# Mbed-TLS/mbedtls

Hardware: AMD Instinct MI355X
Metric: TLS records/sec + GiB/s AEAD throughput (device-resident), 16 KiB records (higher is better)
Workload: dtype u8

## Files before the change

### mbedtls_amd/csrc/tlsrec_device.h

```cpp
#ifndef TLSREC_DEVICE_H
#define TLSREC_DEVICE_H

#include <hip/hip_runtime.h>
#include <stdint.h>

namespace tlsrec {

struct SboxGen {
    uint8_t v[256];
    constexpr SboxGen() : v() {
        uint8_t ex[256] = {};
        uint8_t lg[256] = {};
        uint8_t x = 1;
        for (int i = 0; i < 255; i++) {
            ex[i] = x;
            lg[x] = (uint8_t) i;
            uint8_t x2 = (uint8_t) ((x << 1) ^ ((x & 0x80) ? 0x1b : 0));
            x = (uint8_t) (x2 ^ x);
        }
        for (int a = 0; a < 256; a++) {
            uint8_t inv = a ? ex[(255 - lg[a]) % 255] : 0;
            uint8_t s = inv, r = inv;
            for (int k = 0; k < 4; k++) {
                r = (uint8_t) ((r << 1) | (r >> 7));
// ... 318 lines not shown
        return cam_encrypt<NR, OFF>(lds, lb, rk, in);
    else
        return aria_encrypt<NR, OFF>(lds, lb, rk, in);
}

template <int NR, bool ARIA, typename RK>
__device__ __forceinline__ uint4 blk_encrypt(const uint8_t *lds, uint32_t lb, RK rk, uint4 in)
{
    if constexpr (ARIA)
        return alt_encrypt<NR, 0>(lds, lb, rk, in);
    else
        return aes_encrypt<NR, 0>(lds, lb, rk, in);
}

template <int PI, int G = 4, bool MEM = true>
__device__ __forceinline__ uint4 gmul(const uint8_t *lds, uint4 y)
{
    const uint32_t w[4] = { y.x, y.y, y.z, y.w };
    uint4 acc = make_uint4(0, 0, 0, 0);
#pragma unroll
    for (int d = 0; d < 4; d++) {
#pragma unroll
        for (int e = 0; e < 4; e++) {
            const int b = 4 * d + e;
            uint32_t ahi = (e == 0) ? (w[d] & 0xf0u) : ((w[d] >> (8 * e)) & 0xf0u);
            uint32_t alo = (e == 0) ? ((w[d] << 4) & 0xf0u) : ((w[d] >> (8 * e - 4)) & 0xf0u);
            uint4 th = *reinterpret_cast<const uint4 *>(lds + ahi + PI * 8192 + (2 * b) * 256);
            uint4 tl = *reinterpret_cast<const uint4 *>(lds + alo + PI * 8192 + (2 * b + 1) * 256);
            acc.x = xor3(acc.x, th.x, tl.x);
            acc.y = xor3(acc.y, th.y, tl.y);
            acc.z = xor3(acc.z, th.z, tl.z);
            acc.w = xor3(acc.w, th.w, tl.w);
        }
        if ((d + 1) % (4 / G) == 0) {
            if constexpr (MEM)
                asm volatile("" : "+v"(acc.x), "+v"(acc.y), "+v"(acc.z), "+v"(acc.w) : : "memory");
            else
                asm volatile("" : "+v"(acc.x), "+v"(acc.y), "+v"(acc.z), "+v"(acc.w));
        }
    }
    return acc;
}

template <int PI, int NE = 4>
__device__ __forceinline__ void gmul_word(const uint8_t *lds, uint32_t wd, int d, uint4 &acc, int e0 = 0)
{
#pragma unroll
    for (int i = 0; i < NE; i++) {
        const int e = e0 + i;
        const int b = 4 * d + e;
        uint32_t ahi = (e == 0) ? (wd & 0xf0u) : ((wd >> (8 * e)) & 0xf0u);
        uint32_t alo = (e == 0) ? ((wd << 4) & 0xf0u) : ((wd >> (8 * e - 4)) & 0xf0u);
        uint4 th = *reinterpret_cast<const uint4 *>(lds + ahi + PI * 8192 + (2 * b) * 256);
        uint4 tl = *reinterpret_cast<const uint4 *>(lds + alo + PI * 8192 + (2 * b + 1) * 256);
        acc.x = xor3(acc.x, th.x, tl.x);
        acc.y = xor3(acc.y, th.y, tl.y);
        acc.z = xor3(acc.z, th.z, tl.z);
        acc.w = xor3(acc.w, th.w, tl.w);
    }
}

#ifndef TLSREC_GH_OR
#define TLSREC_GH_OR 1
#endif
template <int PI, int NE = 4>
__device__ __forceinline__ void gmul_word_or(const uint8_t *lds, uint32_t base, uint32_t wd, int d, uint4 &acc,
                                             int e0 = 0)
{
#pragma unroll
    for (int i = 0; i < NE; i++) {
        const int e = e0 + i;
        const int b = 4 * d + e;
        const uint32_t ahi = base | ((e == 0) ? (wd & 0xf0u) : ((wd >> (8 * e)) & 0xf0u));
        const uint32_t alo = base | ((e == 0) ? ((wd << 4) & 0xf0u) : ((wd >> (8 * e - 4)) & 0xf0u));
        uint4 th = *reinterpret_cast<const uint4 *>(lds + ahi + PI * 8192 + (2 * b) * 256);
        uint4 tl = *reinterpret_cast<const uint4 *>(lds + alo + PI * 8192 + (2 * b + 1) * 256);
        acc.x = xor3(acc.x, th.x, tl.x);
        acc.y = xor3(acc.y, th.y, tl.y);
        acc.z = xor3(acc.z, th.z, tl.z);
        acc.w = xor3(acc.w, th.w, tl.w);
    }
}

constexpr int G5_HI = 26 * 256;
struct G5Win { uint8_t d, s, cross; };
__host__ __device__ constexpr G5Win g5_win(int k)
{
    return k < 6 ? G5Win{ 0, (uint8_t) (5 * k), 0 }
         : k == 6 ? G5Win{ 0, 30, 1 }
         : k < 13 ? G5Win{ 1, (uint8_t) (2 + 5 * (k - 7)), 0 }
         : k < 19 ? G5Win{ 2, (uint8_t) (5 * (k - 13)), 0 }
         : k == 19 ? G5Win{ 2, 30, 1 }
         : G5Win{ 3, (uint8_t) (2 + 5 * (k - 20)), 0 };
}
__host__ __device__ constexpr int g5_word(int k, int i) { return g5_win(k).cross && i >= 2 ? g5_win(k).d + 1 : g5_win(k).d; }
__host__ __device__ constexpr int g5_bit(int k, int i)
{
    return g5_win(k).cross ? (i < 2 ? 30 + i : i - 2) : g5_win(k).s + i;
}
__host__ __device__ constexpr int g5_bits(int k) { return g5_win(k).cross ? 4 : 5; }

template <int K>
__device__ __forceinline__ uint32_t g5_addr(const uint32_t (&w)[4])
{
    constexpr G5Win W = g5_win(K);
    if constexpr (W.cross)
        return __builtin_amdgcn_alignbit(w[W.d + 1], w[W.d], 27) & 0x78u;
    else if constexpr (W.s >= 3)
        return (w[W.d] >> (W.s - 3)) & 0xF8u;
    else
        return (w[W.d] << (3 - W.s)) & 0xF8u;
}

__device__ __forceinline__ uint32_t g5_hi(uint32_t a)
{
    uint32_t h;
    asm("v_mov_b32 %0, %1" : "=v"(h) : "v"(a));
    return h;
}

template <int K0, int NK>
__device__ __forceinline__ void gmul5_part(const uint8_t *lds, const uint32_t (&w)[4], uint4 &acc)
{
    if constexpr (NK >= 2) {
        const uint32_t a0 = g5_addr<K0>(w), a1 = g5_addr<K0 + 1>(w);
        const uint2 l0 = *reinterpret_cast<const uint2 *>(lds + a0 + K0 * 256);
        const uint2 h0 = *reinterpret_cast<const uint2 *>(lds + g5_hi(a0) + G5_HI + K0 * 256);
        const uint2 l1 = *reinterpret_cast<const uint2 *>(lds + a1 + (K0 + 1) * 256);
        const uint2 h1 = *reinterpret_cast<const uint2 *>(lds + g5_hi(a1) + G5_HI + (K0 + 1) * 256);
        acc.x = xor3(acc.x, l0.x, l1.x);
        acc.y = xor3(acc.y, l0.y, l1.y);
        acc.z = xor3(acc.z, h0.x, h1.x);
        acc.w = xor3(acc.w, h0.y, h1.y);
        gmul5_part<K0 + 2, NK - 2>(lds, w, acc);
    } else if constexpr (NK == 1) {
        const uint32_t a0 = g5_addr<K0>(w);
        const uint2 l0 = *reinterpret_cast<const uint2 *>(lds + a0 + K0 * 256);
        const uint2 h0 = *reinterpret_cast<const uint2 *>(lds + g5_hi(a0) + G5_HI + K0 * 256);
        acc.x ^= l0.x;
        acc.y ^= l0.y;
        acc.z ^= h0.x;
        acc.w ^= h0.y;
    }
}

template <int G>
__device__ __forceinline__ void gmul5_phase(const uint8_t *lds, const uint32_t (&w)[4], uint4 &acc)
{
    constexpr int K0 = G < 2 ? 4 * G : 8 + 3 * (G - 2);
    constexpr int NK = G < 2 ? 4 : 3;
    gmul5_part<K0, NK>(lds, w, acc);
}

__device__ __forceinline__ uint4 gmul5(const uint8_t *lds, uint4 y)
{
    const uint32_t w[4] = { y.x, y.y, y.z, y.w };
    uint4 acc = make_uint4(0, 0, 0, 0);
    gmul5_part<0, 7>(lds, w, acc);
    asm volatile("" : "+v"(acc.x), "+v"(acc.y), "+v"(acc.z), "+v"(acc.w) : : "memory");
    gmul5_part<7, 6>(lds, w, acc);
    asm volatile("" : "+v"(acc.x), "+v"(acc.y), "+v"(acc.z), "+v"(acc.w) : : "memory");
    gmul5_part<13, 7>(lds, w, acc);
    asm volatile("" : "+v"(acc.x), "+v"(acc.y), "+v"(acc.z), "+v"(acc.w) : : "memory");
    gmul5_part<20, 6>(lds, w, acc);
    return acc;
}

template <int AES_OFF, typename RK>
__device__ __forceinline__ void aes_round(const uint8_t *lds, uint32_t lb, RK rk, int r,
                                          uint32_t &s0, uint32_t &s1, uint32_t &s2, uint32_t &s3)
{
    uint32_t t0 = xor3(tlook<AES_OFF>(lds, s0, lb, 0, 0), tlook<AES_OFF>(lds, s1, lb, 1, 1),
                       rotl16(xor3(tlook<AES_OFF>(lds, s2, lb, 2, 0), tlook<AES_OFF>(lds, s3, lb, 3, 1), rk[4 * r + 0])));
    uint32_t t1 = xor3(tlook<AES_OFF>(lds, s1, lb, 0, 0), tlook<AES_OFF>(lds, s2, lb, 1, 1),
                       rotl16(xor3(tlook<AES_OFF>(lds, s3, lb, 2, 0), tlook<AES_OFF>(lds, s0, lb, 3, 1), rk[4 * r + 1])));
    uint32_t t2 = xor3(tlook<AES_OFF>(lds, s2, lb, 0, 0), tlook<AES_OFF>(lds, s3, lb, 1, 1),
                       rotl16(xor3(tlook<AES_OFF>(lds, s0, lb, 2, 0), tlook<AES_OFF>(lds, s1, lb, 3, 1), rk[4 * r + 2])));
    uint32_t t3 = xor3(tlook<AES_OFF>(lds, s3, lb, 0, 0), tlook<AES_OFF>(lds, s0, lb, 1, 1),
                       rotl16(xor3(tlook<AES_OFF>(lds, s1, lb, 2, 0), tlook<AES_OFF>(lds, s2, lb, 3, 1), rk[4 * r + 3])));
    s0 = t0; s1 = t1; s2 = t2; s3 = t3;
}

struct CtrCache { uint32_t k0r, k1r, d0, d1, d2r, d3; };

template <int AES_OFF, typename RK>
__device__ __forceinline__ CtrCache ctr_cache(const uint8_t *lds, uint32_t lb, RK rk, uint32_t n0, uint32_t n1,
                                              uint32_t n2)
{
#define TA(x, k) tlook<AES_OFF>(lds, (x), lb, (k), 0)
#define TB(x, k) tlook<AES_OFF>(lds, (x), lb, (k), 1)
    const uint32_t s0 = n0 ^ rk[0], s1 = n1 ^ rk[1], s2 = n2 ^ rk[2], s3 = rk[3];
    CtrCache c;
    c.k0r = rotr16(xor3(TA(s0, 0), TB(s1, 1), rotl16(TA(s2, 2) ^ rk[4])));
    c.k1r = rotr16(xor3(TA(s1, 0), TB(s2, 1), rotl16(TB(s0, 3) ^ rk[5])));
    const uint32_t t2 = xor3(TA(s2, 0), TB(s3, 1), rotl16(xor3(TA(s0, 2), TB(s1, 3), rk[6])));
    const uint32_t t3 = xor3(TA(s3, 0), TB(s0, 1), rotl16(xor3(TA(s1, 2), TB(s2, 3), rk[7])));
    c.d0 = rotl16(xor3(TA(t2, 2), TB(t3, 3), rk[8]));
    c.d1 = TB(t2, 1) ^ rotl16(TA(t3, 2) ^ rk[9]);
    c.d2r = rotr16(TA(t2, 0) ^ TB(t3, 1)) ^ rk[10];
    c.d3 = TA(t3, 0) ^ rotl16(TB(t2, 3) ^ rk[11]);
    return c;
#undef TA
#undef TB
}

template <int NR, int AES_OFF, int PI, int R0 = 2, int RS = 1, bool G5 = false, typename RK>
__device__ __forceinline__ void aes_ghash(const uint8_t *lds, const uint8_t *gh, uint32_t lb, RK rk,
                                          const CtrCache &cc, uint32_t ctrw, uint4 y, uint4 &ks, uint4 &prod)
{
    static_assert(R0 >= 2 && R0 + 7 * RS <= NR - 1, "GHASH groups must fall on middle rounds 2..NR-1");
#define TA(x, k) tlook<AES_OFF>(lds, (x), lb, (k), 0)
#define TB(x, k) tlook<AES_OFF>(lds, (x), lb, (k), 1)
    uint32_t s0, s1, s2, s3;
    {
        const uint32_t w3 = ctrw ^ rk[3];
        const uint32_t t0 = rotl16(cc.k0r ^ TB(w3, 3));
        const uint32_t t1 = rotl16(cc.k1r ^ TA(w3, 2));
        s0 = xor3(TA(t0, 0), TB(t1, 1), cc.d0);
        s1 = xor3(TA(t1, 0), cc.d1, rotl16(TB(t0, 3)));
        s2 = rotl16(xor3(TA(t0, 2), TB(t1, 3), cc.d2r));
        s3 = xor3(TB(t0, 1), cc.d3, rotl16(TA(t1, 2)));
    }
#undef TA
#undef TB
    uint32_t w[4] = { y.x, y.y, y.z, y.w };
    uint4 acc = make_uint4(0, 0, 0, 0);
#pragma unroll
    for (int r = 2; r < NR; r++) {
        if (r > 2) aes_round<AES_OFF>(lds, lb, rk, r, s0, s1, s2, s3);
        const int g = (r - R0) / RS;
        if (r >= R0 && (r - R0) % RS == 0 && g < 8) {
            if constexpr (G5) {
                switch (g) {
                    case 0: gmul5_phase<0>(gh, w, acc); break;
                    case 1: gmul5_phase<1>(gh, w, acc); break;
                    case 2: gmul5_phase<2>(gh, w, acc); break;
                    case 3: gmul5_phase<3>(gh, w, acc); break;
                    case 4: gmul5_phase<4>(gh, w, acc); break;
                    case 5: gmul5_phase<5>(gh, w, acc); break;
                    case 6: gmul5_phase<6>(gh, w, acc); break;
                    default: gmul5_phase<7>(gh, w, acc); break;
                }
                asm volatile("" : "+v"(s0), "+v"(s1), "+v"(s2), "+v"(s3), "+v"(acc.x), "+v"(acc.y), "+v"(acc.z),
                             "+v"(acc.w));
                if (g < 2) asm volatile("" : "+v"(w[0]), "+v"(w[1]), "+v"(w[2]), "+v"(w[3]));
                else if (g < 4) asm volatile("" : "+v"(w[1]), "+v"(w[2]), "+v"(w[3]));
                else if (g < 6) asm volatile("" : "+v"(w[2]), "+v"(w[3]));
                else asm volatile("" : "+v"(w[3]));
            } else {
                if constexpr (TLSREC_GH_OR)
                    gmul_word_or<PI, 2>(lds, (uint32_t) (gh - lds), w[g >> 1], g >> 1, acc, 2 * (g & 1));
                else
                    gmul_word<PI, 2>(gh, w[g >> 1], g >> 1, acc, 2 * (g & 1));
                asm volatile("" : "+v"(s0), "+v"(s1), "+v"(s2), "+v"(s3), "+v"(acc.x), "+v"(acc.y), "+v"(acc.z),
                             "+v"(acc.w));
                if (g < 2) asm volatile("" : "+v"(w[1]), "+v"(w[2]), "+v"(w[3]));
                else if (g < 4) asm volatile("" : "+v"(w[2]), "+v"(w[3]));
                else if (g < 6) asm volatile("" : "+v"(w[3]));
            }
        }
    }
    uint32_t o[4];
    const uint32_t s[4] = { s0, s1, s2, s3 };
#pragma unroll
    for (int c = 0; c < 4; c++) {
        uint32_t a = tlook<AES_OFF>(lds, s[c], lb, 0, 0);
        uint32_t b = tlook<AES_OFF>(lds, s[(c + 1) & 3], lb, 1, 0);
        uint32_t d2 = tlook<AES_OFF>(lds, s[(c + 2) & 3], lb, 2, 0);
        uint32_t d3 = tlook<AES_OFF>(lds, s[(c + 3) & 3], lb, 3, 0);
        uint32_t lo = __builtin_amdgcn_perm(b, a, 0x0C0C0501u);
        uint32_t hi = __builtin_amdgcn_perm(d3, d2, 0x06020C0Cu);
        o[c] = __builtin_amdgcn_bitop3_b32(lo, hi, rk[4 * NR + c], 0x56);
    }
    ks = make_uint4(o[0], o[1], o[2], o[3]);
    prod = acc;
}

template <int NR, int AES_OFF, int PI, int NB, typename RK>
__device__ __forceinline__ void aes_ghash_n(const uint8_t *lds, uint32_t lb, RK rk, const CtrCache &cc,
                                            const uint32_t (&ctrw)[NB], const uint4 (&y)[NB], uint4 (&ks)[NB],
                                            uint4 (&prod)[NB])
{
    static_assert(NR >= 10, "rounds 2..9 carry the GHASH groups");
#define TA(x, k) tlook<AES_OFF>(lds, (x), lb, (k), 0)
#define TB(x, k) tlook<AES_OFF>(lds, (x), lb, (k), 1)
    uint32_t s[NB][4];
    uint32_t w[NB][4];
    uint4 acc[NB];
#pragma unroll
    for (int b = 0; b < NB; b++) {
        const uint32_t w3 = ctrw[b] ^ rk[3];
        const uint32_t t0 = rotl16(cc.k0r ^ TB(w3, 3));
        const uint32_t t1 = rotl16(cc.k1r ^ TA(w3, 2));
        s[b][0] = xor3(TA(t0, 0), TB(t1, 1), cc.d0);
        s[b][1] = xor3(TA(t1, 0), cc.d1, rotl16(TB(t0, 3)));
        s[b][2] = rotl16(xor3(TA(t0, 2), TB(t1, 3), cc.d2r));
        s[b][3] = xor3(TB(t0, 1), cc.d3, rotl16(TA(t1, 2)));
        w[b][0] = y[b].x; w[b][1] = y[b].y; w[b][2] = y[b].z; w[b][3] = y[b].w;
        acc[b] = make_uint4(0, 0, 0, 0);
    }
#undef TA
#undef TB
#pragma unroll
    for (int r = 2; r < NR; r++) {
        if (r > 2) {
#pragma unroll
            for (int b = 0; b < NB; b++) aes_round<AES_OFF>(lds, lb, rk, r, s[b][0], s[b][1], s[b][2], s[b][3]);
        }
        const int g = r - 2;
        if (g < 8) {
#pragma unroll
            for (int b = 0; b < NB; b++) gmul_word<PI, 2>(lds, w[b][g >> 1], g >> 1, acc[b], 2 * (g & 1));
#pragma unroll
            for (int b = 0; b < NB; b++) {
                asm volatile("" : "+v"(s[b][0]), "+v"(s[b][1]), "+v"(s[b][2]), "+v"(s[b][3]), "+v"(acc[b].x),
                             "+v"(acc[b].y), "+v"(acc[b].z), "+v"(acc[b].w));
                if (g < 2) asm volatile("" : "+v"(w[b][1]), "+v"(w[b][2]), "+v"(w[b][3]));
                else if (g < 4) asm volatile("" : "+v"(w[b][2]), "+v"(w[b][3]));
                else if (g < 6) asm volatile("" : "+v"(w[b][3]));
            }
        }
    }
#pragma unroll
    for (int b = 0; b < NB; b++) {
        uint32_t o[4];
#pragma unroll
        for (int c = 0; c < 4; c++) {
            uint32_t a = tlook<AES_OFF>(lds, s[b][c], lb, 0, 0);
            uint32_t bb = tlook<AES_OFF>(lds, s[b][(c + 1) & 3], lb, 1, 0);
            uint32_t d2 = tlook<AES_OFF>(lds, s[b][(c + 2) & 3], lb, 2, 0);
            uint32_t d3 = tlook<AES_OFF>(lds, s[b][(c + 3) & 3], lb, 3, 0);
            uint32_t lo = __builtin_amdgcn_perm(bb, a, 0x0C0C0501u);
            uint32_t hi = __builtin_amdgcn_perm(d3, d2, 0x06020C0Cu);
            o[c] = __builtin_amdgcn_bitop3_b32(lo, hi, rk[4 * NR + c], 0x56);
        }
        ks[b] = make_uint4(o[0], o[1], o[2], o[3]);
        prod[b] = acc[b];
    }
}

__device__ __forceinline__ uint4 xor4(uint4 a, uint4 b) { return make_uint4(a.x ^ b.x, a.y ^ b.y, a.z ^ b.z, a.w ^ b.w); }

struct G128 { uint64_t hi, lo; };

__device__ __forceinline__ G128 g_shr1(G128 v)
{
// ... 301 lines not shown
```

### mbedtls_amd/csrc/tlsrec_gcm.h

```cpp
#ifndef TLSREC_GCM_H
#define TLSREC_GCM_H

#include <hip/hip_runtime.h>
#include <stdint.h>
#include <stdlib.h>
#include <type_traits>

#include "tlsrec.h"
#include "tlsrec_clmul.h"
#include "tlsrec_device.h"
#include "tlsrec_frame.h"
#include "tlsrec_internal.h"
#include "tlsrec_recdev.h"

#ifndef TLSREC_GCM_LINE_GROUPS
#define TLSREC_GCM_LINE_GROUPS 1
#endif

#ifndef TLSREC_ABLATE
#define TLSREC_ABLATE 0
#endif
#ifndef TLSREC_PLAN_STASH
#define TLSREC_PLAN_STASH 0
#endif
// ... 62 lines not shown
struct GcmJob {
    bool run, aligned, inner;
    bool wide_tail;
    uint8_t inner_type;
    uint32_t aead_len, content_len, aad_len;
    uint32_t nw0, nw1, nw2;
    uint4 aadw;
    const uint8_t *src;
    uint8_t *dst;

    template <bool DEC>
    __device__ __forceinline__ void setup(const tlsrec_plan &p, const tlsrec_batch_rec &d,
                                          const tlsrec_key_material &km, const uint8_t *in, uint8_t *out)
    {
        uint32_t nw[3];
        nonce_words<DEC>(p, d, km, in, nw);
        nw0 = nw[0]; nw1 = nw[1]; nw2 = nw[2];
        aadw = aad_words(p);
        aad_len = p.aad_len;
        aead_len = p.aead_len;
        content_len = DEC ? p.aead_len : p.content_len;
        inner_type = p.inner_type;
        inner = p.inner;
        src = in + d.buf_off + p.aead_pos;
        dst = out + d.buf_off + p.aead_pos;
        aligned = true;
        wide_tail = true;
        run = true;
    }
};

__device__ __noinline__ uint4 gcm_cid_aad_fold(const uint8_t *gp, uint4 a0, const tlsrec_plan &p,
                                               const tlsrec_batch_rec &d, const uint8_t *cid)
{
    uint4 f = xor4(gmul<0>(gp, a0), cid_aad_block<1, 0>(p, d, cid));
    if (p.aad_len > 32) f = xor4(gmul<0>(gp, f), cid_aad_block<2, 0>(p, d, cid));
    if (p.aad_len > 48) f = xor4(gmul<0>(gp, f), cid_aad_block<3, 0>(p, d, cid));
    return f;
}

__device__ __forceinline__ uint4 gf_mul_i(uint4 x, uint4 p)
{
    const uint32_t a[4] = { x.x, x.y, x.z, x.w }, b[4] = { p.x, p.y, p.z, p.w };
    uint32_t r[4];
    tlsrec_gf128_mul(a, b, r);
    return make_uint4(r[0], r[1], r[2], r[3]);
}
__device__ __noinline__ uint4 gf_mul_v(uint4 x, uint4 p) { return gf_mul_i(x, p); }

template <int SH>
__device__ __forceinline__ uint4 gtree_v(const uint4 (&P)[5], uint4 Y, int lane, int q)
{
    if constexpr (SH >= 1) {
        uint4 o = from_up4<SH>(Y, lane);
        if (q < SH) Y = xor4(gf_mul_v(Y, P[Log2<SH>::v]), o);
        return gtree_v<SH / 2>(P, Y, lane, q);
    } else {
        return Y;
    }
}

template <int SH>
__device__ __forceinline__ uint4 gtree(const uint8_t *lds, uint4 Y, int lane, int q)
{
    if constexpr (SH >= 1) {
        uint4 o = from_up4<SH>(Y, lane);
        if (q < SH) Y = xor4(gmul<Log2<SH>::v>(lds, Y), o);
        return gtree<SH / 2>(lds, Y, lane, q);
    } else {
        return Y;
    }
}

template <int L, int NR, bool DEC, int W, int B, bool WP = false, bool CID = false, bool ARIA = false,
          bool G5 = false, bool PAIR = false>
__global__ __launch_bounds__(W * 64) void tlsrec_gcm_kernel(GcmArgs a)
{
    static_assert(!G5 || (L == 1 << KEY_G5_POWER && !WP && !CID && !ARIA && B == 1), "G5: the 8-lane 16-wave kernel");
    static_assert(!PAIR || (WP && W == 16 && B == 1 && !CID && !ARIA && !G5), "PAIR: 16-wave paired wave passes");
    using LY = GcmLds<L, W, WP, G5, PAIR>;
    constexpr int NTHR = W * 64;
    constexpr int LOGL = Log2<L>::v;
    constexpr int R = 64 / L;
    __shared__ __attribute__((aligned(16))) uint8_t lds[LY::BYTES];
    const int tid = threadIdx.x, wave = tid >> 6, lane = tid & 63;
    const int g = lane / L, q = lane % L;
    const uint32_t lanebase = (uint32_t) (lane & 31) << 2;
    uint32_t *ctl = reinterpret_cast<uint32_t *>(lds + LY::CTL);

    const uint32_t lo = a.perm ? *a.lo : 0u;
    const uint32_t count = a.perm ? *a.hi - lo : (uint32_t) a.n;
    const uint64_t wg_base = (uint64_t) blockIdx.x * W * a.rpw;
    if (wg_base >= count) return;

    if constexpr (ARIA)
        alt_fill_tables<NR>(lds + LY::AES, tid, NTHR);
    else
        aes_fill_tables(lds + LY::AES, tid, NTHR);

    const int pr = wave & (W / 2 - 1), ph = wave / (W / 2);
    const tlsrec_batch_rec *const dsrc = (a.perm && a.srecs) ? a.srecs + lo : a.recs;
    auto membership = [&](uint64_t cb, uint64_t pend, uint32_t &my_slot, uint32_t &my_rec,
                          uint32_t &my_d) __attribute__((always_inline)) {
        {
            const uint64_t pos = PAIR ? cb + 2 * (uint64_t) lane + (uint64_t) ph
                                 : WP ? wg_base + (uint64_t) wave * a.rpw + lane : wg_base + (uint64_t) lane * W + wave;
            if (lane < (int) a.rpw && pos < pend) {
                my_rec = a.perm ? a.perm[lo + pos] : (uint32_t) pos;
                my_d = (a.perm && a.srecs) ? (uint32_t) pos : my_rec;
                const uint32_t s = dsrc[my_d].slot;
                if (TLSREC_HOOK_SKIP(my_rec, a.skip)) {
                } else if (s < a.capacity && a.slots[s].km.cipher == a.cipher) {
                    my_slot = s;
                } else if (!a.perm && !(s < a.capacity && a.slots[s].km.cipher != 0)) {
                    bad_slot_result(a.recs[my_rec], &a.res[my_rec]);
                }
            }
        }
    };
    constexpr int HPI = WP ? 0 : LOGL;
    const uint8_t *hor = WP ? lds + LY::GH + (PAIR ? pr : wave) * 8192 : (G5 ? lds + LY::HG5 : lds + LY::GH);
    constexpr bool EJ0_ONCE = WP || (!G5 && !ARIA);
    uint32_t phase = 0;
    auto passes = [&](uint32_t my_slot, uint32_t my_rec, uint32_t my_d) __attribute__((always_inline)) {
        if constexpr (EJ0_ONCE) {
            uint4 ej0 = make_uint4(0, 0, 0, 0);
            if (my_slot != 0xffffffffu) {
                const SlotState *ss = &a.slots[my_slot];
                const tlsrec_key_material km = ss->km;
                const tlsrec_batch_rec d = dsrc[my_d];
                tlsrec_plan p;
                make_plan<DEC, CID>(p, d, km, ss, a.in);
                uint32_t nw[3];
                nonce_words<DEC>(p, d, km, a.in, nw);
                if constexpr (ARIA)
                    ej0 = alt_encrypt<NR, LY::AES>(lds, lanebase, (const uint32_t *) ss->ark,
                                                   make_uint4(nw[0], nw[1], nw[2], bswap32(1u)));
                else
                    ej0 = aes_encrypt<NR, LY::AES>(lds, lanebase, (const uint32_t *) ss->rkr,
                                                   make_uint4(nw[0], nw[1], nw[2], bswap32(1u)));
            }
            reinterpret_cast<uint4 *>(lds + LY::EJ0)[wave * 64 + lane] = ej0;
        }
        for (int iter = 0;; iter++) {
            uint32_t s;
            if constexpr (PAIR) {
                uint32_t *pmin = ctl + 4 + 2 * pr;
                uint32_t *pcnt = ctl + 20 + pr;
                const uint32_t m = __builtin_amdgcn_readfirstlane(wave_min(my_slot));
                if (lane == 0) pmin[ph] = m;
                pair_sync(pcnt, phase, lane);
                s = __builtin_amdgcn_readfirstlane(min(pmin[0], pmin[1]));
                if (s == 0xffffffffu) break;
                if ((TLSREC_ABLATE & 2) != 0) {
                } else if (a.tm & 16u) {
                    gtab4_build_half(const_cast<uint8_t *>(hor), a.ghtab + (size_t) s * KEY_TABLE_WORDS + KEY_HPOW_OFF + (L - 1),
                                     lane, ph);
                } else {
                    const uint4 *src = a.ghtab + (size_t) s * KEY_TABLE_WORDS + LOGL * 512;
                    uint4 *dst = reinterpret_cast<uint4 *>(const_cast<uint8_t *>(hor));
                    for (int i = lane + ph * 256; i < (ph + 1) * 256; i += 64) dst[i] = src[i];
                }
                pair_sync(pcnt, phase, lane);
            } else if constexpr (WP) {
                s = __builtin_amdgcn_readfirstlane(wave_min(my_slot));
                if (s == 0xffffffffu) break;
// ... 57 lines not shown
                GcmJob jb;
                jb.run = false;
                if (active) {
                    const tlsrec_batch_rec d = dsrc[didx];
                    tlsrec_plan p;
                    make_plan<DEC, CID>(p, d, km, &a.slots[s], a.in);
                    if (p.status != 0) {
                        if (q == 0) finish_early(p, d, a.out, &a.res[ridx]);
                    } else {
                        jb.setup<DEC>(p, d, km, a.in, a.out);
                        if constexpr (PAIR && (TLSREC_PLAN_STASH & (DEC ? 1 : 2)) != 0) {
                            if (q == 0)
                                reinterpret_cast<uint4 *>(lds + LY::FOLD)[wave * LY::FOLDN + g] =
                                    make_uint4(p.data_offset, p.data_len, (uint32_t) p.post_status,
                                               (uint32_t) p.type | ((uint32_t) d.type << 8));
                            if constexpr (!DEC)
                                if (q == 0 && p.explicit_iv && p.post_status == 0) {
                                    uint8_t *e = a.out + d.buf_off + p.data_offset;
                                    for (int i = 0; i < 8; i++) e[i] = d.ctr[i];
                                }
                        }
                        if constexpr (!DEC)
                            if (a.src_off) {
                                jb.src = a.in + a.src_off[ridx];
                                jb.wide_tail = false;
                            }
                        if (CID && p.aad_len > 16) jb.aadw = gcm_cid_aad_fold(gp, jb.aadw, p, d, a.slots[s].cid);
                    }
                }
                const uint32_t m = jb.run ? (jb.aead_len + 15) >> 4 : 0;
                const uint32_t mm = m ? m : 1;
                constexpr uint32_t BL = (uint32_t) (B * L);
                const bool lp = PAIR || (WP && !CID && (a.tm & 8u));
                const bool lenx = lp && m % BL == 0;
                const uint32_t z = lp ? 0u : (BL - mm % BL) % BL;
                const uint32_t J = jb.run ? (lp ? (lenx ? m / BL : (m + BL) / BL) : (mm + z) / BL) : 0;
                const uint32_t Jmax = wave_max(J);
                uint4 *fold = reinterpret_cast<uint4 *>(lds + LY::FOLD) + (PAIR ? wave * LY::FOLDN + g : wave * 64 + lane);
                if (!lp && jb.run && (uint32_t) q == z % L) {
                    uint4 f = jb.aadw;
                    if (m) {
                        if constexpr (WP)
                            f = (a.tm & 4u) ? gf_mul_v(f, h1v) : gmul<0>(gp, f);
                        else
                            f = gmul<0>(gp, f);
                    }
                    *fold = f;
                }
                uint4 Z = make_uint4(0, 0, 0, 0), Xp = make_uint4(0, 0, 0, 0);
                if (lp && jb.run && q == L - 1) Xp = jb.aadw;
                uint32_t nzpos = 0;
                const uint8_t *safe = jb.run ? (jb.wide_tail ? jb.src : jb.dst) : reinterpret_cast<const uint8_t *>(a.recs);
                uint32_t jh = 0;
                {
                    const uint32_t mfast = (jb.run && jb.aligned) ? jb.content_len / 16 : 0;
                    if constexpr (WP && DEC) {
                        uint32_t h = jb.run ? (mfast + z) / BL : 0xffffffffu;
                        h = wave_min(h);
                        if (__ballot(!jb.run)) {
                            constexpr uint32_t hmax = GCM_DUMMY_BYTES / (16 * BL) - 4;
                            h = a.dummy ? (h < hmax ? h : hmax) : 0;
                            if (!jb.run) {
                                jb.src = a.dummy;
                                jb.dst = a.dummy;
                                jb.nw0 = jb.nw1 = jb.nw2 = 0;
                                jb.inner = false;
                            }
                        }
                        jh = h > 1 ? h : 0;
                    } else {
                        uint32_t h = jb.run ? (mfast + z) / BL : 0;
                        h = wave_min(h);
                        jh = h > 1 ? h : 0;
                    }
                }
                const uint32_t jl = jh ? ((DEC && lp) ? 0u : 1u) : Jmax;
                auto steps = [&](auto cached) {
                    constexpr bool CACHED = decltype(cached)::value;
                    CtrCache ccache;
                    if constexpr (CACHED) ccache = ctr_cache<LY::AES>(lds, lanebase, rk, jb.nw0, jb.nw1, jb.nw2);
                    auto crypt = [&](int32_t cc, uint4 y, uint4 &ks, uint4 &Zn) {
                        const uint32_t ctrw = bswap32((uint32_t) cc + 2u);
                        if constexpr (CACHED) {
                            aes_ghash<NR, LY::AES, HPI, 2, 1, G5>(lds, hor, lanebase, rk, ccache, ctrw, y, ks, Zn);
                        } else {
                            if constexpr (ARIA)
                                ks = alt_encrypt<NR, LY::AES>(lds, lanebase, rk, make_uint4(jb.nw0, jb.nw1, jb.nw2, ctrw));
                            else
                                ks = aes_encrypt<NR, LY::AES>(lds, lanebase, rk, make_uint4(jb.nw0, jb.nw1, jb.nw2, ctrw));
                            if constexpr (G5)
                                Zn = gmul5(hor, y);
                            else
                                Zn = gmul<HPI>(hor, y);
                        }
                    };
                    auto general = [&](uint32_t j) {
                        const bool live = jb.run && j < J;
    #pragma unroll
                        for (int b = 0; b < B; b++) {
                            const int32_t cc = (int32_t) (BL * j + L * b + q) - (int32_t) z;
                            const bool valid = live && cc >= 0 && (uint32_t) cc < m;
                            const uint32_t pos = (uint32_t) cc * 16;
                            const bool fast = valid && jb.aligned && pos + 16 <= jb.content_len;
                            uint4 blk = gload16(fast ? jb.src + pos : safe);
                            uint4 ks, Zn;
                            crypt(cc, xor4(Z, Xp), ks, Zn);
                            uint4 X = make_uint4(0, 0, 0, 0);
                            if (fast) {
                                const uint4 o = xor4(blk, ks);
                                gstore16(jb.dst + pos, o);
                                X = DEC ? blk : o;
                                if (DEC && jb.inner && (o.x | o.y | o.z | o.w)) nzpos = pos + 1;
                            } else if (valid) {
                                blk = load_block(jb.src, pos, jb.content_len, jb.aead_len, jb.inner_type,
                                                 jb.aligned && jb.wide_tail);
                                const uint4 o = mask_block(xor4(blk, ks), pos, jb.aead_len);
                                store_block(jb.dst, pos, jb.aead_len, o, jb.aligned);
                                X = DEC ? blk : o;
                                if (DEC && jb.inner && (o.x | o.y | o.z | o.w)) nzpos = pos + 1;
                            }
                            if (lp) {
                                if (cc == (int32_t) m)
                                    X = make_uint4(0, bswap32(jb.aad_len * 8), 0, bswap32(jb.aead_len * 8));
                                if (live && cc <= (int32_t) m) { Z = Zn; Xp = X; }
                            } else {
                                if (live && cc == 0) X = xor4(X, *fold);
                                if (live) { Z = Zn; Xp = X; }
                            }
                        }
                    };
                    uint32_t j = 0;
                    for (; j < jl; j++) general(j);
                    {
                        const uint8_t *sp = jb.src + (size_t) (BL * j + q - z) * 16;
                        uint8_t *dp = jb.dst + (size_t) (BL * j + q - z) * 16;
                        if constexpr ((PAIR || (TLSREC_GCM_LINE_GROUPS & 2)) && L <= 4 && B == 1 &&
                                      (TLSREC_GCM_LINE_GROUPS & 1)) {
                            constexpr int G = 128 / (16 * L);
                            for (; j < jh && j % G != 0; j++) {
                                const int32_t cc = (int32_t) (BL * j + q) - (int32_t) z;
                                const uint4 blk = gload16(sp);
                                uint4 ks, Zn;
                                crypt(cc, xor4(Z, Xp), ks, Zn);
                                const uint4 o = xor4(blk, ks);
                                gstore16(dp, o);
                                if (DEC && jb.inner && (o.x | o.y | o.z | o.w)) nzpos = (uint32_t) cc * 16 + 1;
                                Z = Zn;
                                Xp = DEC ? blk : o;
                                sp += 16 * BL;
                                dp += 16 * BL;
                            }
                            for (; j + G <= jh; j += G) {
                                uint4 blk[G], out[G];
    #pragma unroll
                                for (int t = 0; t < G; t++) blk[t] = gload16(sp + 16 * BL * t);
    #pragma unroll
                                for (int t = 0; t < G; t++) {
                                    const int32_t cc = (int32_t) (BL * (j + t) + q) - (int32_t) z;
                                    uint4 ks, Zn;
                                    crypt(cc, xor4(Z, Xp), ks, Zn);
                                    out[t] = xor4(blk[t], ks);
                                    if (DEC && jb.inner && (out[t].x | out[t].y | out[t].z | out[t].w))
                                        nzpos = (uint32_t) cc * 16 + 1;
                                    Z = Zn;
                                    Xp = DEC ? blk[t] : out[t];
                                }
    #pragma unroll
// ... 302 lines not shown
```

Baseline: 769.0.

## Split fused AES-GHASH rounds into LDS issue and XOR tail phases with wave priority

In the 16-wave non-paired kernel, each fused AES round plus GHASH phase is split into two parts. All LDS table lookups (AES T-table and GHASH table reads) are issued first at raised wave priority via s_setprio, and the XOR reductions run afterwards at normal priority. The last AES round uses the same pattern with perm and bitop3 combining. The aim is to keep the LDS pipe saturated across waves and overlap lookup latency with VALU work, at the cost of more live registers, which may reduce occupancy. A profiling helper script is also added.

```diff
diff --git a/mbedtls_amd/csrc/tlsrec_device.h b/mbedtls_amd/csrc/tlsrec_device.h
--- a/mbedtls_amd/csrc/tlsrec_device.h
+++ b/mbedtls_amd/csrc/tlsrec_device.h
@@ -424,6 +424,32 @@
     }
 }
 
+template <int PI>
+__device__ __forceinline__ void gmul_half_issue(const uint8_t *lds, uint32_t base, uint32_t wd, int d, int e0,
+                                                uint4 (&v)[4])
+{
+#pragma unroll
+    for (int i = 0; i < 2; i++) {
+        const int e = e0 + i;
+        const int b = 4 * d + e;
+        const uint32_t ahi = base | ((e == 0) ? (wd & 0xf0u) : ((wd >> (8 * e)) & 0xf0u));
+        const uint32_t alo = base | ((e == 0) ? ((wd << 4) & 0xf0u) : ((wd >> (8 * e - 4)) & 0xf0u));
+        v[2 * i] = *reinterpret_cast<const uint4 *>(lds + ahi + PI * 8192 + (2 * b) * 256);
+        v[2 * i + 1] = *reinterpret_cast<const uint4 *>(lds + alo + PI * 8192 + (2 * b + 1) * 256);
+    }
+}
+
+__device__ __forceinline__ void gmul_half_tail(const uint4 (&v)[4], uint4 &acc)
+{
+#pragma unroll
+    for (int i = 0; i < 2; i++) {
+        acc.x = xor3(acc.x, v[2 * i].x, v[2 * i + 1].x);
+        acc.y = xor3(acc.y, v[2 * i].y, v[2 * i + 1].y);
+        acc.z = xor3(acc.z, v[2 * i].z, v[2 * i + 1].z);
+        acc.w = xor3(acc.w, v[2 * i].w, v[2 * i + 1].w);
+    }
+}
+
 constexpr int G5_HI = 26 * 256;
 struct G5Win { uint8_t d, s, cross; };
 __host__ __device__ constexpr G5Win g5_win(int k)
@@ -523,6 +549,74 @@
     s0 = t0; s1 = t1; s2 = t2; s3 = t3;
 }
 
+constexpr int PRIO_ISSUE = 3;
+constexpr int PRIO_TAIL = 0;
+
+template <int AES_OFF>
+__device__ __forceinline__ void aes_round_issue(const uint8_t *lds, uint32_t lb, uint32_t s0, uint32_t s1,
+                                                uint32_t s2, uint32_t s3, uint32_t (&v)[16])
+{
+    const uint32_t s[4] = { s0, s1, s2, s3 };
+#pragma unroll
+    for (int c = 0; c < 4; c++) {
+        v[4 * c + 0] = tlook<AES_OFF>(lds, s[c], lb, 0, 0);
+        v[4 * c + 1] = tlook<AES_OFF>(lds, s[(c + 1) & 3], lb, 1, 1);
+        v[4 * c + 2] = tlook<AES_OFF>(lds, s[(c + 2) & 3], lb, 2, 0);
+        v[4 * c + 3] = tlook<AES_OFF>(lds, s[(c + 3) & 3], lb, 3, 1);
+    }
+}
+
+template <typename RK>
+__device__ __forceinline__ void aes_round_tail(RK rk, int r, const uint32_t (&v)[16], uint32_t &s0, uint32_t &s1,
+                                               uint32_t &s2, uint32_t &s3)
+{
+    s0 = xor3(v[0], v[1], rotl16(xor3(v[2], v[3], rk[4 * r + 0])));
+    s1 = xor3(v[4], v[5], rotl16(xor3(v[6], v[7], rk[4 * r + 1])));
+    s2 = xor3(v[8], v[9], rotl16(xor3(v[10], v[11], rk[4 * r + 2])));
+    s3 = xor3(v[12], v[13], rotl16(xor3(v[14], v[15], rk[4 * r + 3])));
+}
+
+template <int K, int K1>
+__device__ __forceinline__ void gmul5_issue_k(const uint8_t *lds, const uint32_t (&w)[4], uint2 (&v)[8])
+{
+    if constexpr (K < K1) {
+        const uint32_t a = g5_addr<K>(w);
+        constexpr int i = 2 * (K1 - 1 - K);
+        v[i] = *reinterpret_cast<const uint2 *>(lds + a + K * 256);
+        v[i + 1] = *reinterpret_cast<const uint2 *>(lds + g5_hi(a) + G5_HI + K * 256);
+        gmul5_issue_k<K + 1, K1>(lds, w, v);
+    }
+}
+
+template <int G>
+__device__ __forceinline__ void gmul5_phase_issue(const uint8_t *lds, const uint32_t (&w)[4], uint2 (&v)[8])
+{
+    constexpr int K0 = G < 2 ? 4 * G : 8 + 3 * (G - 2);
+    constexpr int NK = G < 2 ? 4 : 3;
+    gmul5_issue_k<K0, K0 + NK>(lds, w, v);
+}
+
+template <int G>
+__device__ __forceinline__ void gmul5_phase_tail(const uint2 (&v)[8], uint4 &acc)
+{
+    constexpr int NK = G < 2 ? 4 : 3;
+    acc.x = xor3(acc.x, v[0].x, v[2].x);
+    acc.y = xor3(acc.y, v[0].y, v[2].y);
+    acc.z = xor3(acc.z, v[1].x, v[3].x);
+    acc.w = xor3(acc.w, v[1].y, v[3].y);
+    if constexpr (NK == 4) {
+        acc.x = xor3(acc.x, v[4].x, v[6].x);
+        acc.y = xor3(acc.y, v[4].y, v[6].y);
+        acc.z = xor3(acc.z, v[5].x, v[7].x);
+        acc.w = xor3(acc.w, v[5].y, v[7].y);
+    } else {
+        acc.x ^= v[4].x;
+        acc.y ^= v[4].y;
+        acc.z ^= v[5].x;
+        acc.w ^= v[5].y;
+    }
+}
+
 struct CtrCache { uint32_t k0r, k1r, d0, d1, d2r, d3; };
 
 template <int AES_OFF, typename RK>
@@ -546,14 +640,33 @@
 #undef TB
 }
 
-template <int NR, int AES_OFF, int PI, int R0 = 2, int RS = 1, bool G5 = false, typename RK>
+template <bool G5>
+__device__ __forceinline__ void ghash_phase_fence(int g, uint32_t &s0, uint32_t &s1, uint32_t &s2, uint32_t &s3,
+                                                  uint4 &acc, uint32_t (&w)[4])
+{
+    asm volatile("" : "+v"(s0), "+v"(s1), "+v"(s2), "+v"(s3), "+v"(acc.x), "+v"(acc.y), "+v"(acc.z), "+v"(acc.w));
+    if constexpr (G5) {
+        if (g < 2) asm volatile("" : "+v"(w[0]), "+v"(w[1]), "+v"(w[2]), "+v"(w[3]));
+        else if (g < 4) asm volatile("" : "+v"(w[1]), "+v"(w[2]), "+v"(w[3]));
+        else if (g < 6) asm volatile("" : "+v"(w[2]), "+v"(w[3]));
+        else asm volatile("" : "+v"(w[3]));
+    } else {
+        if (g < 2) asm volatile("" : "+v"(w[1]), "+v"(w[2]), "+v"(w[3]));
+        else if (g < 4) asm volatile("" : "+v"(w[2]), "+v"(w[3]));
+        else if (g < 6) asm volatile("" : "+v"(w[3]));
+    }
+}
+
+template <int NR, int AES_OFF, int PI, int R0 = 2, int RS = 1, bool G5 = false, bool PHASE = false, typename RK>
 __device__ __forceinline__ void aes_ghash(const uint8_t *lds, const uint8_t *gh, uint32_t lb, RK rk,
                                           const CtrCache &cc, uint32_t ctrw, uint4 y, uint4 &ks, uint4 &prod)
 {
     static_assert(R0 >= 2 && R0 + 7 * RS <= NR - 1, "GHASH groups must fall on middle rounds 2..NR-1");
+    static_assert(!PHASE || (R0 == 2 && RS == 1), "PHASE: one GHASH phase per round from round 2");
 #define TA(x, k) tlook<AES_OFF>(lds, (x), lb, (k), 0)
 #define TB(x, k) tlook<AES_OFF>(lds, (x), lb, (k), 1)
     uint32_t s0, s1, s2, s3;
+    if constexpr (PHASE) __builtin_amdgcn_s_setprio(PRIO_ISSUE);
     {
         const uint32_t w3 = ctrw ^ rk[3];
         const uint32_t t0 = rotl16(cc.k0r ^ TB(w3, 3));
@@ -569,8 +682,46 @@
     uint4 acc = make_uint4(0, 0, 0, 0);
 #pragma unroll
     for (int r = 2; r < NR; r++) {
+        const int g = (r - R0) / RS;
+        if constexpr (PHASE) {
+            uint32_t tv[16];
+            uint2 g5v[8];
+            uint4 g4v[4];
+            if (r > 2) {
+                __builtin_amdgcn_s_setprio(PRIO_ISSUE);
+                aes_round_issue<AES_OFF>(lds, lb, s0, s1, s2, s3, tv);
+            }
+            if (g < 8) {
+                if constexpr (G5) {
+                    switch (g) {
+                        case 0: gmul5_phase_issue<0>(gh, w, g5v); break;
+                        case 1: gmul5_phase_issue<1>(gh, w, g5v); break;
+                        case 2: gmul5_phase_issue<2>(gh, w, g5v); break;
+                        case 3: gmul5_phase_issue<3>(gh, w, g5v); break;
+                        case 4: gmul5_phase_issue<4>(gh, w, g5v); break;
+                        case 5: gmul5_phase_issue<5>(gh, w, g5v); break;
+                        case 6: gmul5_phase_issue<6>(gh, w, g5v); break;
+                        default: gmul5_phase_issue<7>(gh, w, g5v); break;
+                    }
+                } else {
+                    gmul_half_issue<PI>(TLSREC_GH_OR ? lds : gh, TLSREC_GH_OR ? (uint32_t) (gh - lds) : 0u, w[g >> 1],
+                                        g >> 1, 2 * (g & 1), g4v);
+                }
+            }
+            __builtin_amdgcn_s_setprio(PRIO_TAIL);
+            if (r > 2) aes_round_tail(rk, r, tv, s0, s1, s2, s3);
+            if (g < 8) {
+                if constexpr (G5) {
+                    if (g < 2) gmul5_phase_tail<0>(g5v, acc);
+                    else gmul5_phase_tail<2>(g5v, acc);
+                } else {
+                    gmul_half_tail(g4v, acc);
+                }
+                ghash_phase_fence<G5>(g, s0, s1, s2, s3, acc, w);
+            }
+            continue;
+        }
         if (r > 2) aes_round<AES_OFF>(lds, lb, rk, r, s0, s1, s2, s3);
-        const int g = (r - R0) / RS;
         if (r >= R0 && (r - R0) % RS == 0 && g < 8) {
             if constexpr (G5) {
                 switch (g) {
@@ -583,27 +734,38 @@
                     case 6: gmul5_phase<6>(gh, w, acc); break;
                     default: gmul5_phase<7>(gh, w, acc); break;
                 }
-                asm volatile("" : "+v"(s0), "+v"(s1), "+v"(s2), "+v"(s3), "+v"(acc.x), "+v"(acc.y), "+v"(acc.z),
-                             "+v"(acc.w));
-                if (g < 2) asm volatile("" : "+v"(w[0]), "+v"(w[1]), "+v"(w[2]), "+v"(w[3]));
-                else if (g < 4) asm volatile("" : "+v"(w[1]), "+v"(w[2]), "+v"(w[3]));
-                else if (g < 6) asm volatile("" : "+v"(w[2]), "+v"(w[3]));
-                else asm volatile("" : "+v"(w[3]));
             } else {
                 if constexpr (TLSREC_GH_OR)
                     gmul_word_or<PI, 2>(lds, (uint32_t) (gh - lds), w[g >> 1], g >> 1, acc, 2 * (g & 1));
                 else
                     gmul_word<PI, 2>(gh, w[g >> 1], g >> 1, acc, 2 * (g & 1));
-                asm volatile("" : "+v"(s0), "+v"(s1), "+v"(s2), "+v"(s3), "+v"(acc.x), "+v"(acc.y), "+v"(acc.z),
-                             "+v"(acc.w));
-                if (g < 2) asm volatile("" : "+v"(w[1]), "+v"(w[2]), "+v"(w[3]));
-                else if (g < 4) asm volatile("" : "+v"(w[2]), "+v"(w[3]));
-                else if (g < 6) asm volatile("" : "+v"(w[3]));
             }
+            ghash_phase_fence<G5>(g, s0, s1, s2, s3, acc, w);
         }
     }
     uint32_t o[4];
     const uint32_t s[4] = { s0, s1, s2, s3 };
+    if constexpr (PHASE) {
+        uint32_t fv[16];
+        __builtin_amdgcn_s_setprio(PRIO_ISSUE);
+#pragma unroll
+        for (int c = 0; c < 4; c++) {
+            fv[4 * c + 0] = tlook<AES_OFF>(lds, s[c], lb, 0, 0);
+            fv[4 * c + 1] = tlook<AES_OFF>(lds, s[(c + 1) & 3], lb, 1, 0);
+            fv[4 * c + 2] = tlook<AES_OFF>(lds, s[(c + 2) & 3], lb, 2, 0);
+            fv[4 * c + 3] = tlook<AES_OFF>(lds, s[(c + 3) & 3], lb, 3, 0);
+        }
+        __builtin_amdgcn_s_setprio(PRIO_TAIL);
+#pragma unroll
+        for (int c = 0; c < 4; c++) {
+            uint32_t lo = __builtin_amdgcn_perm(fv[4 * c + 1], fv[4 * c + 0], 0x0C0C0501u);
+            uint32_t hi = __builtin_amdgcn_perm(fv[4 * c + 3], fv[4 * c + 2], 0x06020C0Cu);
+            o[c] = __builtin_amdgcn_bitop3_b32(lo, hi, rk[4 * NR + c], 0x56);
+        }
+        ks = make_uint4(o[0], o[1], o[2], o[3]);
+        prod = acc;
+        return;
+    }
 #pragma unroll
     for (int c = 0; c < 4; c++) {
         uint32_t a = tlook<AES_OFF>(lds, s[c], lb, 0, 0);
diff --git a/mbedtls_amd/csrc/tlsrec_gcm.h b/mbedtls_amd/csrc/tlsrec_gcm.h
--- a/mbedtls_amd/csrc/tlsrec_gcm.h
+++ b/mbedtls_amd/csrc/tlsrec_gcm.h
@@ -168,6 +168,7 @@
     constexpr int NTHR = W * 64;
     constexpr int LOGL = Log2<L>::v;
     constexpr int R = 64 / L;
+    constexpr bool KP = !WP && !PAIR && !CID && !ARIA && W == 16;
     __shared__ __attribute__((aligned(16))) uint8_t lds[LY::BYTES];
     const int tid = threadIdx.x, wave = tid >> 6, lane = tid & 63;
     const int g = lane / L, q = lane % L;
@@ -391,7 +392,7 @@
                     auto crypt = [&](int32_t cc, uint4 y, uint4 &ks, uint4 &Zn) {
                         const uint32_t ctrw = bswap32((uint32_t) cc + 2u);
                         if constexpr (CACHED) {
-                            aes_ghash<NR, LY::AES, HPI, 2, 1, G5>(lds, hor, lanebase, rk, ccache, ctrw, y, ks, Zn);
+                            aes_ghash<NR, LY::AES, HPI, 2, 1, G5, KP>(lds, hor, lanebase, rk, ccache, ctrw, y, ks, Zn);
                         } else {
                             if constexpr (ARIA)
                                 ks = alt_encrypt<NR, LY::AES>(lds, lanebase, rk, make_uint4(jb.nw0, jb.nw1, jb.nw2, ctrw));
diff --git a/profiles/wave_step.py b/profiles/wave_step.py
--- /dev/null
+++ b/profiles/wave_step.py
@@ -0,0 +1,25 @@
+#!/usr/bin/env python3
+import json
+import sys
+
+s = json.load(open(sys.argv[1]))
+blocks = int(sys.argv[2])
+sq1, sq2, sq3 = s["pmc_sq1"], s["pmc_sq2"], s["pmc_sq3"]
+steps = s["derived"]["records_per_dispatch"] * blocks / 64
+q = 4.0 / steps
+out = {
+    "wave_steps_per_dispatch": steps,
+    "lds_busy_cycles": sq3["SQ_LDS_IDX_ACTIVE"] / steps,
+    "wave_cycles": sq1["SQ_WAVE_CYCLES"] * q,
+    "issue_cycles": sq2["SQ_ACTIVE_INST_ANY"] * q,
+    "valu_cycles": sq2["SQ_ACTIVE_INST_VALU"] * q,
+    "lds_issue_cycles": sq2["SQ_ACTIVE_INST_LDS"] * q,
+    "wait_issue_cycles": sq2["SQ_WAIT_INST_ANY"] * q,
+    "wait_issue_lds_cycles": sq1["SQ_WAIT_INST_LDS"] * q,
+    "waitcnt_cycles": sq2["SQ_WAIT_ANY"] * q,
+    "valu_insts": sq1["SQ_INSTS_VALU"] / steps,
+    "lds_insts": sq1["SQ_INSTS_LDS"] / steps,
+}
+out["lds_busy_frac_resident"] = 16 * out["lds_busy_cycles"] / out["wave_cycles"]
+out["lds_busy_frac"] = s["derived"]["lds_busy_frac"]
+print(json.dumps({k: round(v, 4) if v < 10 else round(v, 1) for k, v in out.items()}, indent=1))
```

Result: faster. 797.1, median of 6 (+3.7%).
